# vandenheuvel/relp

Measured on AMD Instinct MI355X. Metric: simplex pivots/sec + wall-clock to optimal, Netlib 25fv47 @1 GPU, higher is better.
Workload: dtype f64; 1 GPU; Netlib 25FV47 821x1876, steepest-edge pricing, explicit-inverse carry, exact certificate inside the timed step, no presolve (+520 virtual artificials); carry=explicit, refactors=0, parallelism=1 LP per GPU x1, certified=True, objective_bits=1791

## Files before the change

### relp_amd/csrc/kernels.hip

```cpp
#include <hip/hip_runtime.h>
#include <hip/hip_ext.h>

#include <cmath>
#include <cstdlib>
#include <string>
#include <utility>

#include "kernels.hpp"
#include "pivot_step.hpp"
#include "price_step.hpp"
#include "solver.hpp"
#include "wave_ops.hpp"

namespace relp {


__global__ void budget_kernel(Ctl* ctl, long long add) {
    if (ctl->status == ST_BUDGET) ctl->status = ST_RUNNING;
    ctl->budget = ctl->iters + add;
}

typedef double f64x2_t __attribute__((ext_vector_type(2)));
template <int RULE, bool USE_LDS, int LPC, bool UNIT = false>
__global__ void __launch_bounds__(256) price_kernel(DeviceLP lp, int skip_weights, double tol_dual, int col_first,
// ... 2304 lines not shown
    const double r_j = __shfl(o_p, lane_p) / alpha_pq;
    double* c_new = t_new + (size_t)j_own * ld;
    double w_j = 0.0;
#pragma unroll
    for (int u = 0; u < KF_U; ++u) {
        const int i = lane + u * WAVE;
        const double a = s_alpha[i];
        w_j += a * o[u];
        if (i < m) c_new[i] = (i == p) ? r_j : ((a != 0.0) ? o[u] - a * r_j : o[u]);
    }
    w_j = wave_sum(w_j);
    if (lane == LAST) {
        lp.w[j_own] = w_j;
        lp.rho[j_own] = r_j;
        lp.minus_pi[j_own] = pi_old - cbar_q * r_j;
    }
    FSTAMP(6);
}
#undef FSTAMP
__global__ void __launch_bounds__(256) begin_batch_kernel(DeviceLP lp, long long add) {
    const DeviceLP::State s0 = lp.state[0];
    for (int i = threadIdx.x; i < lp.m; i += 256) {
        s0.xB[i] = lp.xB[i];
        s0.basis[i] = lp.basis[i];
    }
    if (threadIdx.x == 0) {
        Ctl c = *lp.ctl;
        if (c.status == ST_BUDGET) c.status = ST_RUNNING;
        c.budget = c.iters + add;
        *lp.ctl = c;
        *s0.ctl = c;
    }
}
__global__ void __launch_bounds__(256) commit_kernel(DeviceLP lp, int parity) {
    const DeviceLP::State last = lp.state[parity];
    const int t_buf = last.ctl->t_buf;
    const int m = lp.m, ld = lp.ld;
    if (t_buf) {
        const int lane = threadIdx.x & (WAVE - 1);
        for (int j = blockIdx.x * 4 + threadIdx.x / WAVE; j < m; j += gridDim.x * 4) {
            const double* src = lp.Binv2 + (size_t)j * ld;
            double* dst = lp.Binv + (size_t)j * ld;
            for (int i = lane; i < m; i += WAVE) dst[i] = src[i];
        }
    }
    if (blockIdx.x == 0) {
        for (int i = threadIdx.x; i < m; i += 256) {
            lp.xB[i] = last.xB[i];
            lp.basis[i] = last.basis[i];
        }
        if (threadIdx.x == 0) {
            Ctl c = *last.ctl;
            c.t_buf = 0;
            *lp.ctl = c;
        }
    }
}

constexpr int K3_THREADS = 256;
constexpr int K3_CPW = 2;
constexpr int K3_SMALL_NZ = 32;
template <bool EAGER>
__global__ void __launch_bounds__(K3_THREADS) update_kernel(DeviceLP lp) {
    Ctl* ctl = lp.ctl;
    const int m = lp.m, ld = lp.ld;
    const int lane = threadIdx.x & (WAVE - 1);
// ... 664 lines not shown
        RELP_LAUNCH(1, (k2l_ftran_kernel<RULE>), dim3(blocks), dim3(K2L_THREADS), 0, s, d, n_price_blocks, tol_pivot, harris_delta, skip_artificial_rows);
        hipLaunchKernelGGL(k2l_harris_kernel, dim3(blocks), dim3(K2L_THREADS), 0, s, d, blocks, tol_pivot, skip_artificial_rows);
        hipLaunchKernelGGL(k2l_apply_kernel, dim3(blocks), dim3(K2L_THREADS), 0, s, d, blocks);
    } else
        RELP_LAUNCH(1, (ftran_ratio_kernel<RULE>), dim3(1), dim3(K2_THREADS), 0, s, d, n_price_blocks, tol_pivot, harris_delta, skip_artificial_rows, mode);
}

bool fast_k2_available(const DeviceLP& d, int n_price_blocks) { return n_price_blocks <= K2F_MAX_BLOCKS && d.m <= 16 * K2F_THREADS; }

void launch_ftran_ratio(const DeviceLP& d, int rule, int n_price_blocks, double tol_pivot, double harris_delta,
                        int skip_artificial_rows, int mode, int n_alpha_slices, hipStream_t s) {
    if (rule == RELP_PIVOT_STEEPEST_EDGE)
        launch_ftran_ratio_rule<RELP_PIVOT_STEEPEST_EDGE>(d, n_price_blocks, tol_pivot, harris_delta, skip_artificial_rows, mode, n_alpha_slices, s);
    else
        launch_ftran_ratio_rule<RELP_PIVOT_DANTZIG>(d, n_price_blocks, tol_pivot, harris_delta, skip_artificial_rows, mode, n_alpha_slices, s);
}

bool fused_pivot_available(const DeviceLP& d, int n_price_blocks) { return d.m <= KF_MAX_M && n_price_blocks <= K2F_MAX_BLOCKS; }
void launch_pivot_fused(const DeviceLP& d, int rule, int parity, int n_price_blocks, double tol_pivot, double harris_delta,
                        int skip_artificial_rows, hipStream_t s) {
    const dim3 grid((d.m + KF_NW - 1) / KF_NW);
    const bool small = d.m <= 2 * KF_THREADS;
    if (rule == RELP_PIVOT_STEEPEST_EDGE) {
        if (small) RELP_LAUNCH(1, (pivot_fused_kernel<RELP_PIVOT_STEEPEST_EDGE, 2>), grid, dim3(KF_THREADS), 0, s, d, d.state[parity], d.state[parity ^ 1], n_price_blocks, tol_pivot, harris_delta, skip_artificial_rows);
        else RELP_LAUNCH(1, (pivot_fused_kernel<RELP_PIVOT_STEEPEST_EDGE, 4>), grid, dim3(KF_THREADS), 0, s, d, d.state[parity], d.state[parity ^ 1], n_price_blocks, tol_pivot, harris_delta, skip_artificial_rows);
    } else {
        if (small) RELP_LAUNCH(1, (pivot_fused_kernel<RELP_PIVOT_DANTZIG, 2>), grid, dim3(KF_THREADS), 0, s, d, d.state[parity], d.state[parity ^ 1], n_price_blocks, tol_pivot, harris_delta, skip_artificial_rows);
        else RELP_LAUNCH(1, (pivot_fused_kernel<RELP_PIVOT_DANTZIG, 4>), grid, dim3(KF_THREADS), 0, s, d, d.state[parity], d.state[parity ^ 1], n_price_blocks, tol_pivot, harris_delta, skip_artificial_rows);
    }
}
void launch_begin_batch(const DeviceLP& d, long long add, hipStream_t s) {
    hipLaunchKernelGGL(begin_batch_kernel, dim3(1), dim3(256), 0, s, d, add);
}
void launch_commit(const DeviceLP& d, int parity, hipStream_t s) {
    hipLaunchKernelGGL(commit_kernel, dim3(std::min(256, (d.m + 3) / 4)), dim3(256), 0, s, d, parity);
}

void launch_update(const DeviceLP& d, hipStream_t s) {
    const int cols_per_block = (K3_THREADS / WAVE) * K3_CPW;
    const dim3 grid((d.m + cols_per_block - 1) / cols_per_block);
    const dim3 grid_split((d.m + K3_CPW - 1) / K3_CPW);
    if (d.m <= 2048) RELP_LAUNCH(2, (update_kernel<true>), grid, dim3(K3_THREADS), 0, s, d);
    else RELP_LAUNCH(2, (update_kernel<false>), (d.track_touched && d.m <= 16384) ? grid_split : grid, dim3(K3_THREADS), 0, s, d);
}

void launch_budget(const DeviceLP& d, long long add, hipStream_t s) {
    hipLaunchKernelGGL(budget_kernel, dim3(1), dim3(1), 0, s, d.ctl, add);
}

void launch_pi(const DeviceLP& d, hipStream_t s) {
    hipLaunchKernelGGL(cb_kernel, dim3(1), dim3(CB_THREADS), 0, s, d);
    hipLaunchKernelGGL(pi_kernel, dim3((d.m + 3) / 4), dim3(256), 0, s, d);
    hipLaunchKernelGGL(pi_sparse_kernel, dim3((d.m + 255) / 256), dim3(256), 0, s, d);
}
void launch_cb(const DeviceLP& d, hipStream_t s) { hipLaunchKernelGGL(cb_kernel, dim3(1), dim3(CB_THREADS), 0, s, d); }
void launch_k2l_preselected(const DeviceLP& d, double tol_pivot, double harris_delta, int skip_artificial_rows, hipStream_t s) {
    const int blocks = (d.m + K2L_THREADS - 1) / K2L_THREADS;
    hipLaunchKernelGGL(k2l_preselected_kernel, dim3(blocks), dim3(K2L_THREADS), 0, s, d, tol_pivot, harris_delta, skip_artificial_rows);
    hipLaunchKernelGGL(k2l_harris_kernel, dim3(blocks), dim3(K2L_THREADS), 0, s, d, blocks, tol_pivot, skip_artificial_rows);
    hipLaunchKernelGGL(k2l_apply_kernel, dim3(blocks), dim3(K2L_THREADS), 0, s, d, blocks);
}
void launch_xb(const DeviceLP& d, hipStream_t s) {
    hipLaunchKernelGGL(xb_kernel, dim3((d.m + WAVE - 1) / WAVE), dim3(256), 0, s, d);
}
void launch_gamma_init(const DeviceLP& d, int identity, hipStream_t s) {
    hipLaunchKernelGGL(gamma_init_kernel, dim3(d.n - d.n_art), dim3(256), 0, s, d, identity);
// ... 85 lines not shown
```

### relp_amd/csrc/kernels.hpp

```cpp
#pragma once
#include "solver.hpp"

namespace relp {

void launch_price(const DeviceLP& d, int rule, int blocks, size_t lds, bool use_lds, int skip_weights, double tol,
                  int first, int last, int cand_offset, hipStream_t s);
void launch_price_dense(const DeviceLP& d, int blocks, int skip_weights, double tol, int cand_offset, hipStream_t s);
void configure_dense_lds(size_t lds);
int dense_lane_slots(int n_dense);
int dense_lane_ld(int m);
void launch_ftran_partial(const DeviceLP& d, int n_slices, int n_price_blocks, int rule, hipStream_t s);
bool fast_k2_available(const DeviceLP& d, int n_price_blocks);
void arm_launch_timer(int which, hipEvent_t start, hipEvent_t stop);
void take_launch_timer(int which, hipEvent_t* start, hipEvent_t* stop);
void configure_lds(size_t price_lds);
int price_columns_per_block(int ell_w, bool generated);
void launch_ftran_ratio(const DeviceLP& d, int rule, int n_price_blocks, double tol_pivot, double harris_delta,
                        int skip_artificial_rows, int mode, int n_alpha_slices, hipStream_t s);
void launch_update(const DeviceLP& d, hipStream_t s);
bool fused_pivot_available(const DeviceLP& d, int n_price_blocks);
void launch_pivot_fused(const DeviceLP& d, int rule, int parity, int n_price_blocks, double tol_pivot, double harris_delta,
                        int skip_artificial_rows, hipStream_t s);
void launch_begin_batch(const DeviceLP& d, long long add, hipStream_t s);
void launch_commit(const DeviceLP& d, int parity, hipStream_t s);
void launch_budget(const DeviceLP& d, long long add, hipStream_t s);
void launch_pi(const DeviceLP& d, hipStream_t s);
void launch_cb(const DeviceLP& d, hipStream_t s);
void launch_k2l_preselected(const DeviceLP& d, double tol_pivot, double harris_delta, int skip_artificial_rows, hipStream_t s);
void launch_xb(const DeviceLP& d, hipStream_t s);
void launch_gamma_init(const DeviceLP& d, int identity, hipStream_t s);
void launch_identity(double* X, int m, int ld, hipStream_t s);
void launch_scatter(double* X, const long long* index, const double* value, long long count, hipStream_t s);
void launch_residual(const DeviceLP& d, const double* X, double* R, hipStream_t s);
void launch_gemm_polish(const double* X, const double* R, double* C, int m, int ld, const int* row_list, int n_rows, hipStream_t s);
void launch_residual_dense(const DeviceLP& d, double* Bd, const double* T, double* S, const int* row_list, int n_rows, hipStream_t s);
void launch_copy_rows(const double* src, double* dst, int m, int ld, const int* row_list, int n_rows, hipStream_t s);
bool gemm_row_lists_supported();
void launch_alpha_reduce(const DeviceLP& d, int n_slices, hipStream_t s);
int eta_max();
void configure_btran_lds(size_t lds);
void launch_eta_update(const DeviceLP& d, double tol_dual, hipStream_t s);
int btran_pass_blocks();
void launch_eta_consolidate(const DeviceLP& d, hipStream_t s);
void launch_mark_all_touched(const DeviceLP& d, hipStream_t s);
void launch_scaled_basis(const DeviceLP& d, double* T, double scale, hipStream_t s);
void launch_row_scan(const DeviceLP& d, int r, double tol, hipStream_t s);
void launch_ftran_vec(const DeviceLP& d, const int* rows, const double* vals, int nnz, double* out, hipStream_t s);
void launch_btran_vec(const DeviceLP& d, const int* rows, const double* vals, int nnz, double* out, hipStream_t s);
void launch_relative_cost(const DeviceLP& d, double* out, hipStream_t s);

void launch_net_row(const DeviceLP& d, const NetTree& t, int r, double* out, hipStream_t s);

}
```

### relp_amd/csrc/solver.hip

```cpp
#include "kernels.hpp"
#include "solver.hpp"

#include <thread>
#include <algorithm>
#include <chrono>
#include <cmath>
#include <cstring>
#include <limits>

namespace relp {

namespace {
double now_seconds() {
    using clock = std::chrono::steady_clock;
    return std::chrono::duration<double>(clock::now().time_since_epoch()).count();
}
void check_sparse(int nnz, const int* rows, const double* values, int m) {
    if (nnz < 0 || nnz > m) throw std::invalid_argument("nnz out of range");
    if (nnz > 0 && (!rows || !values)) throw std::invalid_argument("null sparse vector");
    for (int e = 0; e < nnz; ++e)
        if (rows[e] < 0 || rows[e] >= m) throw std::invalid_argument("index out of range");
}
template <class T>
void upload_vec(T* dst, const std::vector<T>& src, hipStream_t s) {
    if (!src.empty()) RELP_HIP(hipMemcpyAsync(dst, src.data(), src.size() * sizeof(T), hipMemcpyHostToDevice, s));
}
template <class T>
std::vector<T> pack_dense_lanes(const DeviceMatrix& a, int first_column, int n_dense, int groups, int dense_ld) {
    constexpr int per_piece = 16 / (int)sizeof(T), pieces = (int)sizeof(T);
    const int tiles_per_group = dense_ld / 64;
    std::vector<T> packed((size_t)groups * 16 * dense_ld, T(0));
    for (int jd = 0; jd < n_dense; ++jd)
        for (int e = a.col_start[first_column + jd]; e < a.col_start[first_column + jd + 1]; ++e) {
            const int row = a.row_index[e], within = row % 64, t = within % 16;
            packed[((((size_t)(jd / 16) * tiles_per_group + row / 64) * pieces + t / per_piece) * 64 + 16 * (within / 16) + jd % 16) * per_piece + t % per_piece] = (T)a.value[e];
        }
    return packed;
}
}

Solver::Solver(const relp_options& options) : opt_(options) {
    int count = 0;
    hipError_t err = hipGetDeviceCount(&count);
    if (err != hipSuccess || count <= 0)
        throw DeviceError("no HIP device available (relp_amd has no CPU fallback)");
    if (opt_.device < 0 || opt_.device >= count) throw DeviceError("device ordinal out of range");
    RELP_HIP(hipSetDevice(opt_.device));
    RELP_HIP(hipStreamCreateWithFlags(&stream_, hipStreamNonBlocking));
    RELP_HIP(hipEventCreate(&ev_a_));
    RELP_HIP(hipEventCreate(&ev_b_));
}

Solver::~Solver() {
    (void)hipSetDevice(opt_.device);
    certify_scratch_.release();
    free_device();
    destroy_graphs();
    if (ev_a_) (void)hipEventDestroy(ev_a_);
    if (ev_b_) (void)hipEventDestroy(ev_b_);
    if (ev_snapshot_) (void)hipEventDestroy(ev_snapshot_);
    if (ev_refactored_) (void)hipEventDestroy(ev_refactored_);
    if (refactor_stream_) (void)hipStreamDestroy(refactor_stream_);
    if (d_basis_snapshot_) (void)hipFree(d_basis_snapshot_);
    if (d_probe_) (void)hipFree(d_probe_);
    if (d_flipped_snapshot_) (void)hipFree(d_flipped_snapshot_);
    if (stream_) (void)hipStreamDestroy(stream_);
}

void Solver::free_device() {
    device_memory_.free_all();
    d_ = DeviceLP{};
    net_ = NetTree{};
}

void Solver::reset_stats() { stats_ = relp_stats{}; }

void Solver::load(StandardForm&& form) {
    RELP_HIP(hipSetDevice(opt_.device));
    loaded_ = false;
    phase_ = 0;
    free_device();
    destroy_graphs();
    form_ = std::move(form);
    certify_scratch_.digit_hints[0] = certify_scratch_.digit_hints[1] = 0;
    certify_scratch_.statics.reset();
    try {
        upload();
    } catch (...) {
        free_device();
        throw;
    }
    loaded_ = true;
// ... 289 lines not shown
        configure_dense_lds((size_t)3 * d_.dense_ld * sizeof(double));
    }
    d_.rhs0 = device_alloc<double>(m);
    if (bounded_) {
        const std::vector<double> ub = implicit_upper_bounds(md, cols_);
        zero_width_.assign(n, 0);
        for (int j = 0; j < n; ++j) zero_width_[j] = ub[j] == 0.0 ? 1 : 0;
        d_.ub = device_alloc<double>(n);
        d_.xub = device_alloc<double>(m);
        d_.flipped = device_alloc<int>(n);
        upload_vec(d_.ub, ub, stream_);
        RELP_HIP(hipStreamSynchronize(stream_));
    }
    if (!fast_k2_available(d_, price_blocks_ + dense_blocks_) && (!sw(RELP_SW_K2_SINGLE) || network_)) {
        d_.k2_partd = device_alloc<double>((size_t)8 * ((m + 1023) / 1024));
        d_.k2_parti = device_alloc<int>((size_t)4 * ((m + 1023) / 1024));
    }
    {
        const bool kernels_have_it = lu_mode_ || network_ || fast_k2_available(d_, price_blocks_ + dense_blocks_);
        if (opt_.ratio_rule == RELP_RATIO_TEXTBOOK && !kernels_have_it)
            throw std::invalid_argument("RELP_RATIO_TEXTBOOK: the reference's ratio test is implemented up to 8192 rows (the multi-workgroup ratio test has the two-pass rule only)");
        ratio_textbook_ = opt_.ratio_rule == RELP_RATIO_TEXTBOOK || (opt_.ratio_rule == RELP_RATIO_AUTO && host_.small_integer_data() && kernels_have_it);
    }
    fused_ = !lu_mode_ && !network_ && !bounded_ && !eta_mode_ && n_dense == 0 && ftran_slices_ == 0 && !d_.track_touched && d_.ell_w == ELL_W &&
             fused_pivot_available(d_, price_blocks_) && opt_.pivot_kernels != 1;
    if (fused_) {
        for (int k = 0; k < 2; ++k) {
            d_.state[k].ctl = device_alloc<Ctl>(1);
            d_.state[k].xB = device_alloc<double>(m);
            d_.state[k].basis = device_alloc<int>(m);
        }
        ensure_polish_buffers();
    }
    d_.scratch = device_alloc<double>((size_t)std::max(m, n) * 3 + 16);
    d_.ctl = device_alloc<Ctl>(1);
    d_.dbg = device_alloc<unsigned long long>(64);
    RELP_HIP(hipMemsetAsync(d_.dbg, 0, 64 * sizeof(unsigned long long), stream_));

    upload_vec(d_.col_start, col_start, stream_);
    upload_vec(d_.row_index, row_index, stream_);
    upload_vec(d_.value, value, stream_);
    upload_vec(d_.row_start, row_start, stream_);
    upload_vec(d_.col_index, col_index, stream_);
    upload_vec(d_.row_value, row_value, stream_);
    upload_vec(d_.cost1, cost1, stream_);
    upload_vec(d_.cost2, cost2, stream_);
    upload_vec(d_.rhs, rhs, stream_);
    upload_vec(d_.rhs0, rhs, stream_);
    if (d_.ell_w == 2 && !d_.cost8) {
        d_.prw = device_alloc<double>((size_t)4 * m);
        RELP_HIP(hipMemsetAsync(d_.prw, 0, (size_t)4 * m * sizeof(double), stream_));
    } else if (d_.ell_w == 2) {
        d_.price_unit_pairs = sw(RELP_SW_PRICE_UNIT_PAIRS);
        d_.rho_words = ((m + 127) / 128) * 4;
        if ((size_t)d_.rho_words * 4 > 64 * 1024 || sw(RELP_SW_NO_RHO_BITS) || d_.price_unit_pairs) d_.rho_words = 0;
        if (d_.rho_words) {
            d_.rho_bits = device_alloc<unsigned>((size_t)2 * d_.rho_words);
            RELP_HIP(hipMemsetAsync(d_.rho_bits, 0, (size_t)2 * d_.rho_words * sizeof(unsigned), stream_));
        } else {
            d_.rho_nz = device_alloc<unsigned char>(m);
            RELP_HIP(hipMemsetAsync(d_.rho_nz, 0, m, stream_));
        }
    }
    RELP_HIP(hipMemsetAsync(d_.rho, 0, m * sizeof(double), stream_));
    RELP_HIP(hipMemsetAsync(d_.w, 0, m * sizeof(double), stream_));
    RELP_HIP(hipMemsetAsync(d_.alpha, 0, m * sizeof(double), stream_));
// ... 6 lines not shown
                         (long long)n_dense * m * dense_entry_bytes_;
    if (d_.cost8) stats_.price_bytes = (long long)(n - n_art) * (8 + 1 + 4);
    stats_.update_bytes = network_ ? 0 : (long long)2 * m * m * 8;
    if (network_) net_allocate();
    h_basis_.assign(m, -1);
    h_solution_.assign(md.nr_columns(), 0.0);
    if (opt_.crash) {
        h_row_start_ = row_start;
        h_col_index_ = col_index;
    }
    if (!(lu_mode_ || network_ || opt_.crash)) host_ = DeviceMatrix{};
}

Ctl Solver::read_ctl() {
    RELP_HIP(hipGetLastError());
    Ctl c;
    RELP_HIP(hipMemcpyAsync(&c, d_.ctl, sizeof(Ctl), hipMemcpyDeviceToHost, stream_));
    RELP_HIP(hipStreamSynchronize(stream_));
    if (c.status == ST_REFACTOR_FAILED) {
        ++device_refactor_failures_;
        if (opt_.verbose > 0) {
            int info[LUF_INFO_WORDS];
            RELP_HIP(hipMemcpy(info, lu().device_info(), sizeof(info), hipMemcpyDeviceToHost));
            fprintf(stderr, "[lu] the device refactorisation gave up with status %d (m %d): host fallback\n", info[LUF_STATUS], d_.m);
        }
        c.status = ST_REFACTOR;
        RELP_HIP(hipMemcpyAsync(d_.ctl, &c, sizeof(Ctl), hipMemcpyHostToDevice, stream_));
        RELP_HIP(hipStreamSynchronize(stream_));
        refactor_lu_host(true);
        refactors_--;
        RELP_HIP(hipMemcpyAsync(&c, d_.ctl, sizeof(Ctl), hipMemcpyDeviceToHost, stream_));
        RELP_HIP(hipStreamSynchronize(stream_));
    }
    return c;
}
void Solver::write_ctl(const Ctl& c) {
    RELP_HIP(hipMemcpyAsync(d_.ctl, &c, sizeof(Ctl), hipMemcpyHostToDevice, stream_));
    RELP_HIP(hipStreamSynchronize(stream_));
}

void Solver::begin_phase_one() {
    if (!loaded_) throw std::runtime_error("no LP loaded");
    RELP_HIP(hipSetDevice(opt_.device));
    const int m = d_.m, n = d_.n, n_art = d_.n_art;
    const std::vector<int>& basis = cols_.basis0;
    std::vector<int> pos = cols_.pos0();
    if (bounded_)
        for (int j = n_art; j < n; ++j)
            if (zero_width_[j] && pos[j] < 0) pos[j] = -3;
    upload_vec(d_.basis, basis, stream_);
    upload_vec(d_.pos, pos, stream_);
    RELP_HIP(hipMemcpyAsync(d_.rhs, d_.rhs0, m * sizeof(double), hipMemcpyDeviceToDevice, stream_));
    if (bounded_) {
        std::vector<double> xub(m, std::numeric_limits<double>::infinity());
        upload_vec(d_.xub, xub, stream_);
        RELP_HIP(hipMemsetAsync(d_.flipped, 0, n * sizeof(int), stream_));
        RELP_HIP(hipStreamSynchronize(stream_));
    }
    RELP_HIP(hipMemcpyAsync(d_.xB, d_.rhs, m * sizeof(double), hipMemcpyDeviceToDevice, stream_));
    if (lu_mode_) lu_identity();
    else if (network_) {
        net_upload(net_build(basis, std::vector<int>()));
        if (net_.stats) RELP_HIP(hipMemsetAsync(net_.stats, 0, NS_WORDS * sizeof(unsigned long long), stream_));
    }
    else launch_identity(d_.Binv, m, d_.ld, stream_);
    RELP_HIP(hipMemsetAsync(d_.touched, 0, m * sizeof(int), stream_));
    binv_identity_ = true;
    refactors_ = 0;
    device_refactor_failures_ = 0;
    refactor_seconds_ = 0.0;
    Ctl c{};
// ... 242 lines not shown
            Ctl pending = read_ctl();
            if (pending.pending) {
                pending.status = ST_RUNNING;
                write_ctl(pending);
                RELP_HIP(hipMemcpyAsync(d_.cost, d_.cost1, d_.n * sizeof(double), hipMemcpyDeviceToDevice, stream_));
                enqueue_price(0);
                RELP_HIP(hipMemcpyAsync(d_.cost, d_.cost2, d_.n * sizeof(double), hipMemcpyDeviceToDevice, stream_));
            }
        } else if (gamma_ready_) {
            gamma_ready_ = false;
        } else if (lu_mode_ && !binv_identity_) {
            launch_lu_gamma(d_, lu().device(), stream_);
        } else if (network_ && !binv_identity_) {
            net_set_gamma();
        } else {
            launch_gamma_init(d_, binv_identity_ ? 1 : 0, stream_);
        }
    }
    Ctl c = read_ctl();
    const double minus_obj = c.minus_obj;
    const int touched_count = c.touched_count;
    const long long bound_flips = c.bound_flips;
    c = Ctl{};
    c.minus_obj = minus_obj;
    c.touched_count = touched_count;
    c.bound_flips = bound_flips;
    c.forced_q = c.forced_p = -1;
    c.last_selected = -1;
    c.scan_column = std::numeric_limits<int>::max();
    write_ctl(c);
}

void Solver::launch_pivots(int count, bool forced) {
    if (fused_ && !forced) {
        launch_begin_batch(d_, count, stream_);
        for (int it = 0; it < count; ++it) {
            enqueue_price_fused(it & 1);
            enqueue_pivot_fused(it & 1);
        }
        launch_commit(d_, count & 1, stream_);
        stats_.launches += 2 + 2LL * count;
        stats_.price_launches += count;
        return;
    }
    launch_budget(d_, count, stream_);
    if (network_) {
        for (int it = 0; it < count; ++it) {
            enqueue_price(0);
            net_enqueue_pivot(0);
        }
        stats_.launches += 1 + (long long)net_launches_per_pivot() * count;
        stats_.price_launches += count;
        return;
    }
    if (lu_mode_) {
        for (int it = 0; it < count; ++it) {
            enqueue_price(0);
            enqueue_ftran_ratio(0);
        }
        stats_.launches += 1 + 2LL * count;
        stats_.price_launches += count;
        return;
    }
    for (int it = 0; it < count; ++it) {
        enqueue_price(0, it == 0);
        enqueue_ftran_ratio(0);
        enqueue_update();
        if (eta_mode_ && ((it + 1) % d_.eta_cap == 0 || it + 1 == count)) enqueue_consolidate();
    }
    stats_.launches += 1 + (3LL + (dense_blocks_ > 0) + 2 * (ftran_slices_ > 0)) * count;
    stats_.price_launches += count;
}

void Solver::enqueue_price(int skip_weights, bool first_of_batch) {
    const size_t lds_max = opt_.price_lds_max > 0 ? (size_t)opt_.price_lds_max : (size_t)96 * 1024;
    const bool use_lds = price_lds_ <= lds_max && dense_blocks_ == 0;
    if (price_blocks_ > 0 && (!slack_in_btran_ || first_of_batch))
        launch_price(d_, opt_.pivot_rule, price_blocks_, use_lds ? price_lds_ : 0, use_lds, slack_in_btran_ ? 1 : skip_weights, opt_.tol_dual,
                     sparse_first_, d_.n, 0, stream_);
    if (dense_blocks_ > 0) launch_price_dense(d_, dense_blocks_, skip_weights, opt_.tol_dual, price_blocks_, stream_);
}

void Solver::enqueue_price_fused(int parity) {
    DeviceLP d = d_;
    d.ctl = d_.state[parity].ctl;
    const bool use_lds = price_lds_ <= 160 * 1024 - 1024;
    launch_price(d, opt_.pivot_rule, price_blocks_, use_lds ? price_lds_ : 0, use_lds, 0, opt_.tol_dual, sparse_first_, d_.n, 0, stream_);
}
void Solver::enqueue_pivot_fused(int parity) {
    launch_pivot_fused(d_, opt_.pivot_rule, parity, price_blocks_, opt_.tol_pivot, ratio_delta(), phase_ == 2 ? 1 : 0, stream_);
}

void Solver::enqueue_update() {
    if (eta_mode_) launch_eta_update(d_, opt_.tol_dual, stream_);
    else launch_update(d_, stream_);
}
void Solver::enqueue_consolidate() {
    if (eta_mode_) launch_eta_consolidate(d_, stream_);
}

void Solver::enqueue_ftran_ratio(int mode) {
    const int skip_art = phase_ == 2 ? 1 : 0;
    const int slots = price_blocks_ + dense_blocks_;
    if (network_) {
        net_enqueue_pivot(mode);
        return;
    }
    if (lu_mode_) {
        hipEvent_t start = nullptr, stop = nullptr;
        take_launch_timer(1, &start, &stop);
        launch_lu_pivot(d_, lu().device(), opt_.pivot_rule, slots, opt_.tol_pivot, ratio_delta(), skip_art, mode, refactor_period_, stream_, start, stop);
        return;
    }
    if (ftran_slices_ > 0) {
        launch_ftran_partial(d_, ftran_slices_, slots, opt_.pivot_rule, stream_);
        launch_alpha_reduce(d_, ftran_slices_, stream_);
    }
    launch_ftran_ratio(d_, opt_.pivot_rule, slots, opt_.tol_pivot, ratio_delta(), skip_art, mode, ftran_slices_ > 0 ? 1 : 0, stream_);
}

void Solver::destroy_graphs() {
    for (int k = 0; k < 4; ++k) {
        if (graph_exec_[k]) { (void)hipGraphExecDestroy(graph_exec_[k]); graph_exec_[k] = nullptr; }
        if (graph_[k]) { (void)hipGraphDestroy(graph_[k]); graph_[k] = nullptr; }
        graph_count_[k] = 0;
    }
}

void Solver::build_graph(int count) {
    const int k = graph_index();
    if (graph_exec_[k] && graph_count_[k] == count) return;
    if (graph_exec_[k]) { (void)hipGraphExecDestroy(graph_exec_[k]); graph_exec_[k] = nullptr; }
    if (graph_[k]) { (void)hipGraphDestroy(graph_[k]); graph_[k] = nullptr; }
    long long launches = stats_.launches, price_launches = stats_.price_launches;
    RELP_HIP(hipStreamBeginCapture(stream_, hipStreamCaptureModeRelaxed));
    launch_pivots(count);
    RELP_HIP(hipStreamEndCapture(stream_, &graph_[k]));
    RELP_HIP(hipGraphInstantiate(&graph_exec_[k], graph_[k], nullptr, nullptr, 0));
    stats_.launches = launches;
    stats_.price_launches = price_launches;
    graph_count_[k] = count;
}

void Solver::polish(bool refresh_vectors, bool force) {
    if (lu_mode_) {
        refactor_lu(refresh_vectors);
        return;
    }
    if (network_) {
        if (since_polish_ == 0 && !force && !(opt_.switches & RELP_SW_POLISH_ALWAYS)) return;
        if (refresh_vectors) net_refresh(true, true);
        polish_scale_ = std::min(256, polish_scale_ * 4);
        polishes_++;
        since_polish_ = 0;
        return;
    }
    if (since_polish_ == 0 && !force && !(opt_.switches & RELP_SW_POLISH_ALWAYS)) return;
    const int m = d_.m;
    const bool by_rows = d_.track_touched && gemm_row_lists_supported();
    const int* rows = by_rows ? d_.tlist : nullptr;
    int n_rows = m;
    if (by_rows) n_rows = read_ctl().touched_count;
    if (d_.n_dense > 0) ensure_polish_buffers();
    for (int it = 0; it < 2; ++it) {
        RELP_HIP(hipMemsetAsync(&d_.ctl->residual, 0, sizeof(double), stream_));
        if (by_rows && d_.R) RELP_HIP(hipMemsetAsync(d_.R, 0, (size_t)m * d_.ld * sizeof(double), stream_));
        if (d_.n_dense > 0) launch_residual_dense(d_, d_.Binv2, d_.Binv, d_.R, rows, n_rows, stream_);
        else launch_residual(d_, d_.Binv, d_.R, stream_);
        Ctl c = read_ctl();
// ... 159 lines not shown
        upload_vec(d_.flipped, flipped, stream_);
        upload_vec(d_.rhs, rhs, stream_);
        upload_vec(d_.xub, xub, stream_);
        RELP_HIP(hipStreamSynchronize(stream_));
    }
    upload_vec(d_.basis, basis, stream_);
    upload_vec(d_.pos, pos, stream_);
    Ctl c{};
    c.forced_q = c.forced_p = -1;
    c.last_selected = -1;
    c.scan_column = std::numeric_limits<int>::max();
    write_ctl(c);
    invert_from_scratch();
    if (lu_mode_) launch_lu_xb(d_, lu().device(), stream_);
    else if (network_) net_refresh(true, false);
    else launch_xb(d_, stream_);
    binv_identity_ = false;
    refactors_ = 0;
    refactor_seconds_ = 0.0;
    pivots_[0] = pivots_[1] = 0;
    polishes_ = 0;
    max_residual_ = 0.0;
    since_polish_ = 0;
    polish_scale_ = 1;
    redundant_rows_.clear();
    set_phase(2);
}

long long Solver::iterate(long long count, int* stop_reason) {
    if (phase_ == 0) throw std::runtime_error("no phase started");
    RELP_HIP(hipSetDevice(opt_.device));
    long long done = 0;
    int reason = ST_BUDGET;
    long long iters_before = read_ctl().iters;
    const int full_batch = async_refactor_ ? (opt_.pivots_per_launch > 0 && opt_.pivots_per_launch < 64 ? opt_.pivots_per_launch : 16) : lu_mode_ ? refactor_period_ + 1 : std::max(1, opt_.pivots_per_launch);
    while (done < count) {
        if (async_in_flight_ && hipEventQuery(ev_refactored_) == hipSuccess) finish_async_refactor(iters_before);
        long long room = (!lu_mode_ && opt_.polish_period > 0) ? (long long)opt_.polish_period * polish_scale_ - since_polish_ : count;
        if (room <= 0) { polish(true); continue; }
        int batch = (int)std::min<long long>({count - done, room, (long long)full_batch});
        if (opt_.use_graph && batch == full_batch) {
            build_graph(batch);
            RELP_HIP(hipGraphLaunch(graph_exec_[graph_index()], stream_));
            stats_.launches += 1 + (network_ ? (long long)net_launches_per_pivot() : lu_mode_ ? 2LL : 3LL) * batch;
            stats_.price_launches += batch;
        } else {
            launch_pivots(batch);
        }
        const long long fallbacks_before = device_refactor_failures_;
        Ctl after = read_ctl();
        const bool fell_back = device_refactor_failures_ != fallbacks_before;
        long long made = after.iters - iters_before;
        iters_before = after.iters;
        done += made;
        since_polish_ += made;
        pivots_[phase_ - 1] += made;
        if (made > 0) binv_identity_ = false;
        if (after.status == ST_NO_ENTERING || after.status == ST_UNBOUNDED) { reason = after.status; break; }
        if (after.status == ST_REFACTOR) {
            if (async_in_flight_ && finish_async_refactor(after.iters)) launch_clear_refactor_status(d_, stream_);
            else refactor_lu(true, false);
            continue;
        }
        if (async_refactor_ && !async_in_flight_ && after.status == ST_RUNNING && lu().device().inverse_factors == 4 &&
            since_polish_ + LU_LOG_CAPACITY + full_batch > refactor_period_)
            start_async_refactor(after.iters);
        if (made == 0 && after.status == ST_RUNNING && !fell_back) break;
    }
    if (stop_reason) *stop_reason = reason;
    return done;
}

int Solver::drive_out_artificials() {
    const int m = d_.m;
    std::vector<int> basis(m);
    RELP_HIP(hipMemcpyAsync(basis.data(), d_.basis, m * sizeof(int), hipMemcpyDeviceToHost, stream_));
    RELP_HIP(hipStreamSynchronize(stream_));
    int redundant = 0;
    for (int r = 0; r < m; ++r) {
        if (basis[r] >= d_.n_art) continue;
        Ctl c = read_ctl();
        c.scan_column = std::numeric_limits<int>::max();
        write_ctl(c);
        if (lu_mode_) {
            double* rowvec = d_.scratch + (d_.m + 1) / 2 + 1 + d_.m;
            int* d_slot = reinterpret_cast<int*>(d_.scratch);
            double* d_one = d_.scratch + (d_.m + 1) / 2 + 1;
            const double one = 1.0;
            RELP_HIP(hipMemcpyAsync(d_slot, &r, sizeof(int), hipMemcpyHostToDevice, stream_));
            RELP_HIP(hipMemcpyAsync(d_one, &one, sizeof(double), hipMemcpyHostToDevice, stream_));
            launch_lu_btran(lu().device(), d_slot, d_one, 1, rowvec, stream_);
            launch_lu_row_scan(d_, rowvec, 1e-7, stream_);
        } else if (network_) {
            double* rowvec = d_.scratch + (d_.m + 1) / 2 + 1 + d_.m;
            launch_net_row(d_, net_, r, rowvec, stream_);
            launch_lu_row_scan(d_, rowvec, 1e-7, stream_);
        } else {
            launch_row_scan(d_, r, 1e-7, stream_);
        }
        c = read_ctl();
        if (c.scan_column == std::numeric_limits<int>::max()) {
            redundant_rows_.push_back(r);
            ++redundant;
            continue;
        }
        c.forced_q = c.scan_column;
        c.forced_p = r;
        c.status = ST_RUNNING;
        write_ctl(c);
        RELP_HIP(hipMemsetAsync(d_.xB + r, 0, sizeof(double), stream_));
        launch_pivots(1, true);
        Ctl after = read_ctl();
        if (after.iters == c.iters) throw std::runtime_error("zero-level pivot failed");
        pivots_[0] += 1;
        since_polish_ += 1;
        if (after.status == ST_REFACTOR) refactor_lu(true);
    }
    return redundant;
}

void Solver::solve(relp_result* result) {
    if (!loaded_) throw std::runtime_error("no LP loaded");
    RELP_HIP(hipSetDevice(opt_.device));
    const double t0 = now_seconds();
    relp_result res{};
    exact_objective.clear();
    exact_primal.reset();
    const bool timing = diagnostic("RELP_TIME_SOLVE");
    double t_last = t0;
    auto tick = [&](const char* what) {
        if (!timing) return;
        RELP_HIP(hipStreamSynchronize(stream_));
        const double t = now_seconds();
        fprintf(stderr, "[solve] %-24s %.3f ms\n", what, (t - t_last) * 1e3);
        t_last = t;
    };
    begin_phase_one();
    tick("begin_phase_one");
    const long long cap = opt_.max_pivots > 0 ? opt_.max_pivots : 200LL * (d_.m + d_.n) + 100000;
    int kind = RELP_RESULT_NONE;
    if (phase_ == 1) {
        int reason = 0;
        long long done = iterate(cap, &reason);
        (void)done;
        tick("phase one loop");
        if (reason == ST_UNBOUNDED) throw std::runtime_error("Artificial cost can not be unbounded.");
        if (reason == ST_BUDGET) kind = RELP_RESULT_ITERATION_LIMIT;
        if (kind == RELP_RESULT_NONE) {
            polish(true);
            tick("polish");
            Ctl c = read_ctl();
            std::vector<double> xb(d_.m);
            RELP_HIP(hipMemcpyAsync(xb.data(), d_.xB, d_.m * sizeof(double), hipMemcpyDeviceToHost, stream_));
            RELP_HIP(hipStreamSynchronize(stream_));
            double scale = 1.0;
            for (double v : xb) scale += std::fabs(v);
            if (-c.minus_obj > opt_.tol_feasible * scale) {
                kind = RELP_RESULT_INFEASIBLE;
            } else {
                tick("feasibility check");
                drive_out_artificials();
                tick("drive out artificials");
                set_phase(2);
                tick("set_phase(2)");
            }
        }
    }
    if (kind == RELP_RESULT_NONE) {
        int reason = 0;
        iterate(cap - pivots_[0], &reason);
        tick("phase two loop");
        if (reason == ST_UNBOUNDED) kind = RELP_RESULT_UNBOUNDED;
        else if (reason == ST_NO_ENTERING) {
            kind = RELP_RESULT_FINITE_OPTIMUM;
            polish(true);
            tick("final polish");
        } else kind = RELP_RESULT_ITERATION_LIMIT;
    }
    const int m = d_.m;
    std::vector<int> basis(m);
    std::vector<double> xb(m);
    RELP_HIP(hipMemcpyAsync(basis.data(), d_.basis, m * sizeof(int), hipMemcpyDeviceToHost, stream_));
    RELP_HIP(hipMemcpyAsync(xb.data(), d_.xB, m * sizeof(double), hipMemcpyDeviceToHost, stream_));
    Ctl c = read_ctl();
    for (int i = 0; i < m; ++i)
        if (basis[i] < 0 || basis[i] >= d_.n) throw std::runtime_error("the device returned an invalid basis (row " + std::to_string(i) + ")");
    std::fill(h_solution_.begin(), h_solution_.end(), 0.0);
    if (!bounded_) {
        for (int i = 0; i < m; ++i) {
            h_basis_[i] = cols_.to_provider(basis[i]);
            if (basis[i] >= d_.n_art) h_solution_[basis[i] - d_.n_art] = xb[i];
        }
    } else {
        const MatrixData& md = form_.data;
// ... 540 lines not shown
```

### relp_amd/csrc/solver.hpp

```cpp
#pragma once
#include <cstdlib>
#include <cstring>
#include <cstddef>
#include <hip/hip_runtime.h>

#include <atomic>
#include <memory>
#include <mutex>
#include <stdexcept>
#include <string>
#include <vector>

#include "../../include/relp_amd.h"
#include "device_columns.hpp"
#include "device_memory.hpp"
#include "model.hpp"
#include "lu.hpp"

namespace relp {

struct ExactPrimal;
struct CertifyScratch {
    hipStream_t second = nullptr;
    struct Block {
// ... 261 lines not shown
    bool refactors_on_device() const { return device_refactor_; }
    long long device_refactor_fallbacks() const { return device_refactor_failures_; }
    bool refactors_asynchronously() const { return async_refactor_; }
    long long async_refactors() const { return async_refactors_; }
    long long async_refactors_abandoned() const { return async_abandoned_; }
    double async_worst_residual() const { return async_worst_residual_; }
    std::string exact_objective;
    std::shared_ptr<const ExactPrimal> exact_primal;
    std::string last_error;
    relp_result last_result{};

private:
    void upload();
    void free_device();
    void set_phase(int phase);
    void launch_pivots(int count, bool forced = false);
    void enqueue_price_fused(int parity);
    void enqueue_pivot_fused(int parity);
    bool fused_ = false;
    void enqueue_price(int skip_weights, bool first_of_batch = true);
    bool slack_in_btran_ = false;
    void enqueue_ftran_ratio(int mode);
    void enqueue_update();
    void enqueue_consolidate();
    void build_graph(int count);
    void polish(bool refresh_vectors, bool force = false);
    void invert_from_scratch();
    std::vector<int> explicit_basis(const std::vector<int>& basis, const std::vector<int>& pos) const;
    void resolve_fixed_columns(std::vector<int>& pos);
    std::vector<char> zero_width_;
    void ensure_polish_buffers();
    Ctl read_ctl();
    void write_ctl(const Ctl& c);
    int drive_out_artificials();
    void certify(relp_result* result);
    std::vector<double> net_host_solve(const HostTree& t, bool transposed, const std::vector<double>& v) const;
    CertifyScratch certify_scratch_;
    bool network_ = false;
    NetTree net_;
    void net_allocate();
    HostTree net_build(const std::vector<int>& basis, const std::vector<int>& flipped) const;
    void net_upload(const HostTree& tree);
    HostTree net_download();
    void net_refresh(bool xb, bool pi);
    void net_gamma(const HostTree& tree, const std::vector<int>& pos, std::vector<double>* gamma) const;
    void net_set_gamma();
    bool net_crash(const std::vector<int>& basis);
    void net_certify(relp_result* result);
    int net_launches_per_pivot() const;
    void net_enqueue_pivot(int mode, int parts = 3);
    std::vector<unsigned long long> net_stats_;
    DeviceAllocations device_memory_;
    template <class T>
    T* device_alloc(size_t count) { return device_memory_.alloc<T>(count); }
    void refactor_lu(bool refresh_vectors, bool settle = true);
    void refactor_lu_host(bool refresh_vectors);
    std::vector<ExactWidthRecord> exact_records_;
    bool device_refactor_ = false;
    long long device_refactor_failures_ = 0;
    void lu_identity();
    LuFactors lu_sets_[2];
    int lu_cur_ = 0;
    LuFactors& lu() { return lu_sets_[lu_cur_]; }
    const LuFactors& lu() const { return lu_sets_[lu_cur_]; }
    bool async_refactor_ = false, async_in_flight_ = false;
    hipStream_t refactor_stream_ = nullptr;
    hipEvent_t ev_snapshot_ = nullptr, ev_refactored_ = nullptr;
// ... 81 lines not shown
```

Before: 54540 pivots/s.

## Pipeline fused pivot batches with double-buffered async control readback

Adds a pipelined iteration path that keeps up to two graph-launched pivot batches in flight. Each batch chains its state from the previous one on the device, and the control block is read back asynchronously into pinned host memory and checked with events instead of a blocking read after every batch. It also caches the iteration count to skip control reads, makes control writes asynchronous during drive-out, and reuses a basis already fetched. The cost is speculative extra pivots issued after termination and more complicated state and parity bookkeeping.

```diff
diff --git a/relp_amd/csrc/kernels.hip b/relp_amd/csrc/kernels.hip
--- a/relp_amd/csrc/kernels.hip
+++ b/relp_amd/csrc/kernels.hip
@@ -2360,6 +2360,28 @@
         *s0.ctl = c;
     }
 }
+__global__ void __launch_bounds__(256) open_batches_kernel(DeviceLP lp, int parity) {
+    const DeviceLP::State s = lp.state[parity];
+    for (int i = threadIdx.x; i < lp.m; i += 256) {
+        s.xB[i] = lp.xB[i];
+        s.basis[i] = lp.basis[i];
+    }
+    if (threadIdx.x == 0) *s.ctl = *lp.ctl;
+}
+__global__ void __launch_bounds__(256) next_batch_kernel(DeviceLP lp, int parity, long long add) {
+    const DeviceLP::State from = lp.state[parity], s0 = lp.state[0];
+    if (parity != 0)
+        for (int i = threadIdx.x; i < lp.m; i += 256) {
+            s0.xB[i] = from.xB[i];
+            s0.basis[i] = from.basis[i];
+        }
+    if (threadIdx.x == 0) {
+        Ctl c = *from.ctl;
+        if (c.status == ST_BUDGET) c.status = ST_RUNNING;
+        if (c.status == ST_RUNNING) c.budget = c.iters + add;
+        *s0.ctl = c;
+    }
+}
 __global__ void __launch_bounds__(256) commit_kernel(DeviceLP lp, int parity) {
     const DeviceLP::State last = lp.state[parity];
     const int t_buf = last.ctl->t_buf;
@@ -3090,6 +3112,12 @@
 void launch_begin_batch(const DeviceLP& d, long long add, hipStream_t s) {
     hipLaunchKernelGGL(begin_batch_kernel, dim3(1), dim3(256), 0, s, d, add);
 }
+void launch_open_batches(const DeviceLP& d, int parity, hipStream_t s) {
+    hipLaunchKernelGGL(open_batches_kernel, dim3(1), dim3(256), 0, s, d, parity);
+}
+void launch_next_batch(const DeviceLP& d, int parity, long long add, hipStream_t s) {
+    hipLaunchKernelGGL(next_batch_kernel, dim3(1), dim3(256), 0, s, d, parity, add);
+}
 void launch_commit(const DeviceLP& d, int parity, hipStream_t s) {
     hipLaunchKernelGGL(commit_kernel, dim3(std::min(256, (d.m + 3) / 4)), dim3(256), 0, s, d, parity);
 }
diff --git a/relp_amd/csrc/kernels.hpp b/relp_amd/csrc/kernels.hpp
--- a/relp_amd/csrc/kernels.hpp
+++ b/relp_amd/csrc/kernels.hpp
@@ -22,6 +22,8 @@
 void launch_pivot_fused(const DeviceLP& d, int rule, int parity, int n_price_blocks, double tol_pivot, double harris_delta,
                         int skip_artificial_rows, hipStream_t s);
 void launch_begin_batch(const DeviceLP& d, long long add, hipStream_t s);
+void launch_open_batches(const DeviceLP& d, int parity, hipStream_t s);
+void launch_next_batch(const DeviceLP& d, int parity, long long add, hipStream_t s);
 void launch_commit(const DeviceLP& d, int parity, hipStream_t s);
 void launch_budget(const DeviceLP& d, long long add, hipStream_t s);
 void launch_pi(const DeviceLP& d, hipStream_t s);
diff --git a/relp_amd/csrc/solver.hip b/relp_amd/csrc/solver.hip
--- a/relp_amd/csrc/solver.hip
+++ b/relp_amd/csrc/solver.hip
@@ -49,6 +49,8 @@
     RELP_HIP(hipStreamCreateWithFlags(&stream_, hipStreamNonBlocking));
     RELP_HIP(hipEventCreate(&ev_a_));
     RELP_HIP(hipEventCreate(&ev_b_));
+    RELP_HIP(hipHostMalloc(reinterpret_cast<void**>(&h_ctl_), 3 * sizeof(Ctl), hipHostMallocDefault));
+    for (hipEvent_t* e : {&ev_batch_[0], &ev_batch_[1], &ev_write_}) RELP_HIP(hipEventCreateWithFlags(e, hipEventDisableTiming));
 }
 
 Solver::~Solver() {
@@ -58,6 +60,10 @@
     destroy_graphs();
     if (ev_a_) (void)hipEventDestroy(ev_a_);
     if (ev_b_) (void)hipEventDestroy(ev_b_);
+    if (stream_) (void)hipStreamSynchronize(stream_);
+    for (hipEvent_t e : {ev_batch_[0], ev_batch_[1], ev_write_})
+        if (e) (void)hipEventDestroy(e);
+    if (h_ctl_) (void)hipHostFree(h_ctl_);
     if (ev_snapshot_) (void)hipEventDestroy(ev_snapshot_);
     if (ev_refactored_) (void)hipEventDestroy(ev_refactored_);
     if (refactor_stream_) (void)hipStreamDestroy(refactor_stream_);
@@ -413,6 +419,7 @@
         }
         ensure_polish_buffers();
     }
+    pipeline_ = fused_ && opt_.use_graph && !diagnostic("RELP_NO_PIPELINE");
     d_.scratch = device_alloc<double>((size_t)std::max(m, n) * 3 + 16);
     d_.ctl = device_alloc<Ctl>(1);
     d_.dbg = device_alloc<unsigned long long>(64);
@@ -485,11 +492,26 @@
         RELP_HIP(hipMemcpyAsync(&c, d_.ctl, sizeof(Ctl), hipMemcpyDeviceToHost, stream_));
         RELP_HIP(hipStreamSynchronize(stream_));
     }
+    write_pending_ = false;
+    iters_known_ = true;
+    iters_now_ = c.iters;
     return c;
 }
 void Solver::write_ctl(const Ctl& c) {
     RELP_HIP(hipMemcpyAsync(d_.ctl, &c, sizeof(Ctl), hipMemcpyHostToDevice, stream_));
     RELP_HIP(hipStreamSynchronize(stream_));
+    write_pending_ = false;
+    iters_known_ = true;
+    iters_now_ = c.iters;
+}
+void Solver::write_ctl_async(const Ctl& c) {
+    if (write_pending_) RELP_HIP(hipEventSynchronize(ev_write_));
+    h_ctl_[2] = c;
+    RELP_HIP(hipMemcpyAsync(d_.ctl, &h_ctl_[2], sizeof(Ctl), hipMemcpyHostToDevice, stream_));
+    RELP_HIP(hipEventRecord(ev_write_, stream_));
+    write_pending_ = true;
+    iters_known_ = true;
+    iters_now_ = c.iters;
 }
 
 void Solver::begin_phase_one() {
@@ -798,6 +820,7 @@
 }
 
 void Solver::launch_pivots(int count, bool forced) {
+    iters_known_ = false;
     if (fused_ && !forced) {
         launch_begin_batch(d_, count, stream_);
         for (int it = 0; it < count; ++it) {
@@ -854,6 +877,7 @@
     launch_price(d, opt_.pivot_rule, price_blocks_, use_lds ? price_lds_ : 0, use_lds, 0, opt_.tol_dual, sparse_first_, d_.n, 0, stream_);
 }
 void Solver::enqueue_pivot_fused(int parity) {
+    iters_known_ = false;
     launch_pivot_fused(d_, opt_.pivot_rule, parity, price_blocks_, opt_.tol_pivot, ratio_delta(), phase_ == 2 ? 1 : 0, stream_);
 }
 
@@ -866,6 +890,7 @@
 }
 
 void Solver::enqueue_ftran_ratio(int mode) {
+    iters_known_ = false;
     const int skip_art = phase_ == 2 ? 1 : 0;
     const int slots = price_blocks_ + dense_blocks_;
     if (network_) {
@@ -900,7 +925,15 @@
     if (graph_[k]) { (void)hipGraphDestroy(graph_[k]); graph_[k] = nullptr; }
     long long launches = stats_.launches, price_launches = stats_.price_launches;
     RELP_HIP(hipStreamBeginCapture(stream_, hipStreamCaptureModeRelaxed));
-    launch_pivots(count);
+    if (pipeline_) {
+        launch_next_batch(d_, count & 1, count, stream_);
+        for (int it = 0; it < count; ++it) {
+            enqueue_price_fused(it & 1);
+            enqueue_pivot_fused(it & 1);
+        }
+    } else {
+        launch_pivots(count);
+    }
     RELP_HIP(hipStreamEndCapture(stream_, &graph_[k]));
     RELP_HIP(hipGraphInstantiate(&graph_exec_[k], graph_[k], nullptr, nullptr, 0));
     stats_.launches = launches;
@@ -1126,7 +1159,8 @@
     RELP_HIP(hipSetDevice(opt_.device));
     long long done = 0;
     int reason = ST_BUDGET;
-    long long iters_before = read_ctl().iters;
+    if (pipeline_) return iterate_pipelined(count, stop_reason);
+    long long iters_before = fused_ && iters_known_ ? iters_now_ : read_ctl().iters;
     const int full_batch = async_refactor_ ? (opt_.pivots_per_launch > 0 && opt_.pivots_per_launch < 64 ? opt_.pivots_per_launch : 16) : lu_mode_ ? refactor_period_ + 1 : std::max(1, opt_.pivots_per_launch);
     while (done < count) {
         if (async_in_flight_ && hipEventQuery(ev_refactored_) == hipSuccess) finish_async_refactor(iters_before);
@@ -1165,17 +1199,88 @@
     return done;
 }
 
-int Solver::drive_out_artificials() {
+long long Solver::iterate_pipelined(long long count, int* stop_reason) {
+    const int full = std::max(1, opt_.pivots_per_launch);
+    const int last = full & 1;
+    long long done = 0;
+    int reason = ST_BUDGET;
+    long long iters_before = iters_known_ ? iters_now_ : read_ctl().iters;
+    bool open = false;
+    unsigned issued = 0, retired = 0;
+    auto close = [&]() {
+        if (!open) return;
+        launch_commit(d_, last, stream_);
+        stats_.launches += 1;
+        open = false;
+    };
+    auto account = [&](const Ctl& after) {
+        const long long made = after.iters - iters_before;
+        iters_before = after.iters;
+        done += made;
+        since_polish_ += made;
+        pivots_[phase_ - 1] += made;
+        if (made > 0) binv_identity_ = false;
+        if (after.status == ST_NO_ENTERING || after.status == ST_UNBOUNDED) {
+            reason = after.status;
+            return true;
+        }
+        return made == 0 && after.status == ST_RUNNING;
+    };
+    for (;;) {
+        const long long ahead = (long long)(issued - retired) * full;
+        const long long room = opt_.polish_period > 0 ? (long long)opt_.polish_period * polish_scale_ - since_polish_ : count;
+        const bool fits = done + ahead + full <= count && ahead + full <= room;
+        if (issued - retired < 2 && fits) {
+            build_graph(full);
+            if (!open) {
+                launch_open_batches(d_, last, stream_);
+                stats_.launches += 1;
+                open = true;
+            }
+            RELP_HIP(hipGraphLaunch(graph_exec_[graph_index()], stream_));
+            stats_.launches += 1 + 3LL * full;
+            stats_.price_launches += full;
+            RELP_HIP(hipMemcpyAsync(&h_ctl_[issued & 1], d_.state[last].ctl, sizeof(Ctl), hipMemcpyDeviceToHost, stream_));
+            RELP_HIP(hipEventRecord(ev_batch_[issued & 1], stream_));
+            ++issued;
+            continue;
+        }
+        if (issued != retired) {
+            RELP_HIP(hipGetLastError());
+            RELP_HIP(hipEventSynchronize(ev_batch_[retired & 1]));
+            const Ctl after = h_ctl_[retired & 1];
+            ++retired;
+            if (account(after)) break;
+            continue;
+        }
+        close();
+        if (done >= count) break;
+        if (room <= 0) { polish(true); continue; }
+        launch_pivots((int)std::min<long long>({count - done, room, (long long)full}));
+        if (account(read_ctl())) break;
+    }
+    close();
+    iters_known_ = true;
+    iters_now_ = iters_before;
+    if (stop_reason) *stop_reason = reason;
+    return done;
+}
+
+int Solver::drive_out_artificials(const std::vector<int>* basis_now) {
     const int m = d_.m;
-    std::vector<int> basis(m);
-    RELP_HIP(hipMemcpyAsync(basis.data(), d_.basis, m * sizeof(int), hipMemcpyDeviceToHost, stream_));
-    RELP_HIP(hipStreamSynchronize(stream_));
+    std::vector<int> fetched;
+    if (!basis_now) {
+        fetched.resize(m);
+        RELP_HIP(hipMemcpyAsync(fetched.data(), d_.basis, m * sizeof(int), hipMemcpyDeviceToHost, stream_));
+        RELP_HIP(hipStreamSynchronize(stream_));
+    }
+    const std::vector<int>& basis = basis_now ? *basis_now : fetched;
     int redundant = 0;
     for (int r = 0; r < m; ++r) {
         if (basis[r] >= d_.n_art) continue;
         Ctl c = read_ctl();
         c.scan_column = std::numeric_limits<int>::max();
-        write_ctl(c);
+        write_ctl_async(c);
         if (lu_mode_) {
             double* rowvec = d_.scratch + (d_.m + 1) / 2 + 1 + d_.m;
             int* d_slot = reinterpret_cast<int*>(d_.scratch);
@@ -1201,7 +1306,7 @@
         c.forced_q = c.scan_column;
         c.forced_p = r;
         c.status = ST_RUNNING;
-        write_ctl(c);
+        write_ctl_async(c);
         RELP_HIP(hipMemsetAsync(d_.xB + r, 0, sizeof(double), stream_));
         launch_pivots(1, true);
         Ctl after = read_ctl();
@@ -1243,17 +1348,18 @@
         if (kind == RELP_RESULT_NONE) {
             polish(true);
             tick("polish");
+            std::vector<double> xb(d_.m);
+            std::vector<int> basis_now(d_.m);
+            RELP_HIP(hipMemcpyAsync(xb.data(), d_.xB, d_.m * sizeof(double), hipMemcpyDeviceToHost, stream_));
+            RELP_HIP(hipMemcpyAsync(basis_now.data(), d_.basis, d_.m * sizeof(int), hipMemcpyDeviceToHost, stream_));
             Ctl c = read_ctl();
-            std::vector<double> xb(d_.m);
-            RELP_HIP(hipMemcpyAsync(xb.data(), d_.xB, d_.m * sizeof(double), hipMemcpyDeviceToHost, stream_));
-            RELP_HIP(hipStreamSynchronize(stream_));
             double scale = 1.0;
             for (double v : xb) scale += std::fabs(v);
             if (-c.minus_obj > opt_.tol_feasible * scale) {
                 kind = RELP_RESULT_INFEASIBLE;
             } else {
                 tick("feasibility check");
-                drive_out_artificials();
+                drive_out_artificials(&basis_now);
                 tick("drive out artificials");
                 set_phase(2);
                 tick("set_phase(2)");
diff --git a/relp_amd/csrc/solver.hpp b/relp_amd/csrc/solver.hpp
--- a/relp_amd/csrc/solver.hpp
+++ b/relp_amd/csrc/solver.hpp
@@ -317,7 +317,16 @@
     void ensure_polish_buffers();
     Ctl read_ctl();
     void write_ctl(const Ctl& c);
-    int drive_out_artificials();
+    void write_ctl_async(const Ctl& c);
+    int drive_out_artificials(const std::vector<int>* basis_now = nullptr);
+    long long iterate_pipelined(long long count, int* stop_reason);
+    bool pipeline_ = false;
+    Ctl* h_ctl_ = nullptr;
+    hipEvent_t ev_batch_[2] = {nullptr, nullptr};
+    hipEvent_t ev_write_ = nullptr;
+    bool write_pending_ = false;
+    bool iters_known_ = false;
+    long long iters_now_ = 0;
     void certify(relp_result* result);
     std::vector<double> net_host_solve(const HostTree& t, bool transposed, const std::vector<double>& v) const;
     CertifyScratch certify_scratch_;
```

New measurement: 54730 pivots/s (median of 4 runs). No clear change (+0.3%).
